# ahcorde/visualSLAM_Android

Hardware: AMD Instinct MI355X
Metric: frames/sec (TrackFrame+local BA) on 640×480 synthetic, 1/2/4/8 GPU (higher is better)
Workload: dtype f64

## Files before the change

visualslam_android_amd/csrc/patch_dev.h:

```cpp
#pragma once
#include "vslam_internal.h"

template <int PS> struct PRow { unsigned w[(PS + 3) / 4]; };
template <int PS> DEVFN PRow<PS> zero_row() {
  PRow<PS> r;
#pragma unroll
  for (int k = 0; k < (PS + 3) / 4; k++) r.w[k] = 0u;
  return r;
}
template <int PS> DEVFN PRow<PS> load_row(const uint8_t* p) {
  PRow<PS> r = zero_row<PS>();
  __builtin_memcpy(&r, p, PS);
  return r;
}
template <int PS> DEVFN PRow<PS> load_row_lds(const uint8_t* p) {
  PRow<PS> r = zero_row<PS>();
#pragma unroll
  for (int x = 0; x < PS; x++) r.w[x >> 2] |= (unsigned)p[x] << (8 * (x & 3));
  return r;
}
template <int PS> DEVFN int row_byte(const PRow<PS>& r, int x) { return (int)((r.w[x >> 2] >> (8 * (x & 3))) & 255u); }
DEVFN unsigned udot4(unsigned a, unsigned b, unsigned c) { return __builtin_amdgcn_udot4(a, b, c, false); }

template <int NPIX> DEVFN int zmssd_score(int tsum, int tsumsq, int sA, int sQ, int sX) {
  const int SA = tsum, SB = sA;
  return ((2 * SA * SB - SA * SA - SB * SB) / NPIX + sQ + tsumsq - 2 * sX);
}
template <int PS, int G> DEVFN void grp_zmssd_sums(const PRow<PS>& row, const PRow<PS>& trow, int& sA, int& sQ, int& sX) {
  unsigned a = 0, q = 0, x = 0;
#pragma unroll
  for (int k = 0; k < (PS + 3) / 4; k++) {
    a = udot4(row.w[k], 0x01010101u, a);
    q = udot4(row.w[k], row.w[k], q);
    x = udot4(row.w[k], trow.w[k], x);
  }
  sA = (int)grp_sum<G>(a); sQ = (int)grp_sum<G>(q); sX = (int)grp_sum<G>(x);
}
template <int PS>
DEVFN int wave_zmssd(const uint8_t* tmpl, const uint8_t* img, int ip, int wl, int hl, int cx, int cy, int tsum, int tsumsq, int max_ssd, int lane) {
  constexpr int NPIX = PS * PS, HALF = PS / 2;
  if (!(cx >= HALF && cy >= HALF && cx < wl - HALF && cy < hl - HALF)) return max_ssd + 1;
  int sA = 0, sQ = 0, sX = 0;
  for (int q = lane; q < NPIX; q += 64) {
    const int y = q / PS, x = q - y * PS;
    const int n = img[(size_t)(cy - HALF + y) * ip + (cx - HALF + x)], t = tmpl[q];
    sA += n; sQ += n * n; sX += n * t;
  }
  sA = wave_sum(sA); sQ = wave_sum(sQ); sX = wave_sum(sX);
  return zmssd_score<NPIX>(tsum, tsumsq, sA, sQ, sX);
}

DEVFN int search_level_and_warp(const Pose& pose, const double cam[3], const double d[4], const double right[3], const double down[3],
                                double warp_inv[4], int& search_level) {
  const double ooz = 1.0 / cam[2];
  double mr[3], md[3];
  pose_rot(pose, right, mr);
  pose_rot(pose, down, md);
  const double r0 = mr[0] - cam[0] * mr[2] * ooz, r1 = mr[1] - cam[1] * mr[2] * ooz;
  const double d0 = md[0] - cam[0] * md[2] * ooz, d1 = md[1] - cam[1] * md[2] * ooz;
  warp_inv[0] = (d[0] * r0 + d[1] * r1) * ooz; warp_inv[2] = (d[2] * r0 + d[3] * r1) * ooz;
  warp_inv[1] = (d[0] * d0 + d[1] * d1) * ooz; warp_inv[3] = (d[2] * d0 + d[3] * d1) * ooz;
  double det = warp_inv[0] * warp_inv[3] - warp_inv[1] * warp_inv[2];
  int lv = 0;
  while (det > 3 && lv < NLEV - 1) { lv++; det *= 0.25; }
  search_level = lv;
  return (det > 3 || det < 0.25) ? -1 : lv;
}

DEVFN void template_warp_matrix(const double warp_inv[4], int scale, double m2[4]) {
  double inv[4];
  inv2(warp_inv, inv);
  m2[0] = inv[0] * scale; m2[1] = inv[1] * scale; m2[2] = inv[2] * scale; m2[3] = inv[3] * scale;
}
DEVFN bool warp_moved(const double m2[4], const double last_warp[4]) {
  for (int i = 0; i < 2; i++) {
    const double dx = m2[i] - last_warp[i], dy = m2[2 + i] - last_warp[2 + i];
    if (dx * dx + dy * dy > 0.07 * 0.07) return true;
  }
  return false;
}
struct TemplateWarp {
  double across[2], down[2], cr[2], x0, y0;
  float x_bound, y_bound;
};
template <int PS> DEVFN TemplateWarp template_warp(const double m2[4], int irx, int iry, int iw, int ih) {
  constexpr int HALF = PS / 2;
  TemplateWarp w;
  w.across[0] = m2[0]; w.across[1] = m2[2]; w.down[0] = m2[1]; w.down[1] = m2[3];
  w.x0 = (double)irx - (m2[0] * HALF + m2[1] * HALF); w.y0 = (double)iry - (m2[2] * HALF + m2[3] * HALF);
  w.cr[0] = w.down[0] - PS * w.across[0]; w.cr[1] = w.down[1] - PS * w.across[1];
  w.x_bound = (float)(iw - 1); w.y_bound = (float)(ih - 1);
  return w;
}
DEVFN void warp_pixel_step(const TemplateWarp& w, double& x, double& y) { x += w.across[0]; y += w.across[1]; }
template <int PS> DEVFN void warp_row_step(const TemplateWarp& w, double& x, double& y) {
#pragma unroll
  for (int j = 0; j < PS; j++) warp_pixel_step(w, x, y);
  x += w.cr[0]; y += w.cr[1];
}
DEVFN int warp_sample(const TemplateWarp& w, const uint8_t* src, int sp, double x, double y, int& nOutside) {
  if (0 <= x && 0 <= y && x < w.x_bound && y < w.y_bound) {
    const int lx = (int)x, ly = (int)y;
    x -= lx; y -= ly;
    const uint8_t* q0 = src + (size_t)ly * sp + lx;
    return (uint8_t)((1 - y) * ((1 - x) * q0[0] + x * q0[1]) + y * ((1 - x) * q0[sp] + x * q0[sp + 1]));
  }
  nOutside++;
  return 0;
}

struct CoarseWindow {
  unsigned range;
  int top, bottom_plus_one, left, right;
  bool empty;
};
DEVFN CoarseWindow coarse_window(double irx, double iry, int range_l0, int scale, int rows) {
  CoarseWindow cw;
  cw.range = ((unsigned)range_l0 + scale - 1) / scale;
  cw.top = (int)(iry - cw.range);
// ... 39 lines not shown
```

visualslam_android_amd/csrc/track.hip:

```cpp
#include "vslam_internal.h"
#include "patch_dev.h"
#include "pvs_perm.h"

#define TRK_THREADS 256
#define SORT_CAP 4096
static_assert(SORT_CAP == PVS_SORT_CAP, "a level's list (at most max_points entries) fits the permutation's sort buffer");

template <class T>
DEVFN bool td_project(T& td, int& flags, const double* pos, const Pose& pose, const CamModel& cam, CamProj& pr) {
  flags &= ~TDF_IN_IMAGE;
  double c[3];
  pose_xform(pose, pos, c);
  td.cam[0] = c[0]; td.cam[1] = c[1]; td.cam[2] = c[2];
  if (c[2] < 0.001) return false;
  const double implane[2] = {c[0] / c[2], c[1] / c[2]};
  if (implane[0] * implane[0] + implane[1] * implane[1] > cam.largest_radius * cam.largest_radius) return false;
  pr = cam_project(cam, implane[0], implane[1]);
  td.image[0] = pr.im[0]; td.image[1] = pr.im[1];
  if (pr.invalid) return true;
  if (td.image[0] < 0 || td.image[1] < 0 || td.image[0] > cam.size[0] || td.image[1] > cam.size[1]) return true;
  flags |= TDF_IN_IMAGE;
  return true;
}

template <class T>
DEVFN void td_project_and_derivs(T& td, int& flags, const double* pos, const Pose& pose, const CamModel& cam) {
  CamProj pr;
  const bool projected = td_project(td, flags, pos, pose, cam, pr);
  if ((flags & TDF_FOUND) && projected) cam_derivs(cam, pr, td.derivs);
}

template <class T>
DEVFN void td_calc_jacobian(const T& td, double* jac) {
  const double ooz = 1.0 / td.cam[2];
  const double c[3] = {td.cam[0], td.cam[1], td.cam[2]};
  const double d0 = td.derivs[0], d1 = td.derivs[1], d2 = td.derivs[2], d3 = td.derivs[3];
#pragma unroll
  for (int m = 0; m < 6; m++) {
    double f0, f1;
    se3_generator_motion(m, c, ooz, f0, f1);
    jac[m] = d0 * f0 + d1 * f1;
    jac[6 + m] = d2 * f0 + d3 * f1;
  }
}

#ifdef VSLAM_PVS_OCC8
#define VSLAM_PVS_ATTR __attribute__((amdgpu_waves_per_eu(8, 8)))
#else
#define VSLAM_PVS_ATTR
#endif
#define PVS_OUT 13
struct PvsOut { double cam[3], image[2], derivs[4], warp_inv[4]; };
static_assert(sizeof(PvsOut) == PVS_OUT * 8 && sizeof(MapPointDev) == PVS_OUT * 8 && sizeof(MapPointDev) % 8 == 0, "one LDS buffer serves both directions");
static_assert(offsetof(TrackData, derivs) == 40 && offsetof(TrackData, warp_inv) == 96, "k_pvs's write-out indexes TrackData as doubles");
__global__ __launch_bounds__(64) void k_motion(MapDev m, int S, const double* sbi_rot ) {
  const int s = blockIdx.x * 64 + threadIdx.x;
  if (s >= S) return;
  if (!trk_in_step(m.held, s)) return;
  TrackerState* st = &m.st[s];
  const bool tracking = trk_runs_track_map(m.held, s, st);
  st->frame++;
  st->kf_pending = 0; st->kf_added = 0;
  if (!tracking) return;
  if (!st->recovered_now) {
    double v[6];
    for (int i = 0; i < 6; i++) v[i] = st->velocity[i];
    if (sbi_rot) { v[0] = 0.0; v[1] = 0.0; for (int i = 3; i < 6; i++) v[i] = sbi_rot[(size_t)s * 8 + i]; }
    const Pose pred = pose_mul(se3_exp(v), st->pose_final);
    st->start_pose = st->pose_final; st->pose_cur = pred;
  }
  for (int l = 0; l < NLEV; l++) { st->attempted[l] = 0; st->found[l] = 0; }
  st->n_search = 0; st->n_coarse = 0; st->n_iter = 0; st->n_l3 = 0; st->coarse_found = 0;
}

__global__ __launch_bounds__(TRK_THREADS) VSLAM_PVS_ATTR void k_pvs(MapDev m, TrackParams tp) {
  const int s = blockIdx.y;
  TrackerState* st = &m.st[s];
  const bool tracking = trk_runs_track_map(m.held, s, st);
  const int n_points = st->n_points, i0 = blockIdx.x * TRK_THREADS;
  if (!tracking || i0 >= n_points) return;
  __shared__ __align__(16) double pbuf[TRK_THREADS * PVS_OUT];
  __shared__ int wn[TRK_THREADS];
  const int nhere = min(TRK_THREADS, n_points - i0);
  {
    const double* src = (const double*)(m.pts + (size_t)s * tp.max_points + i0);
    for (int k = threadIdx.x; k < nhere * PVS_OUT; k += TRK_THREADS) pbuf[k] = src[k];
  }
  const Pose pred = st->pose_cur;
  __syncthreads();
  const int i = i0 + threadIdx.x;
  PvsOut td;
  int nwr = 0;
  if (i < n_points) {
    const MapPointDev p = *(const MapPointDev*)(pbuf + (size_t)threadIdx.x * PVS_OUT);
    const size_t gi = (size_t)s * tp.max_points + i;
    int level = -1;
    if (!p.bad) {
      int flags = m.pt_flags[gi];
      CamProj pr;
      const bool projected = td_project(td, flags, p.pos, pred, tp.cam, pr);
      nwr = projected ? 5 : 3;
      if (flags & TDF_IN_IMAGE) {
        nwr = PVS_OUT;
        cam_derivs(tp.cam, pr, td.derivs);
        int lv;
        level = search_level_and_warp(pred, td.cam, td.derivs, p.right, p.down, td.warp_inv, lv);
        if (level < 0) flags |= TDF_TMPL_BAD;
        else flags &= ~(TDF_SEARCHED | TDF_FOUND);
      }
      m.pt_flags[gi] = flags;
    }
    m.pt_level[gi] = level;
  }
  __syncthreads();
  wn[threadIdx.x] = nwr;
  {
    const double* t = (const double*)&td;
    for (int f = 0; f < PVS_OUT; f++) if (f < nwr) pbuf[threadIdx.x * PVS_OUT + f] = t[f];
  }
  __syncthreads();
  double* dst = (double*)(m.td + (size_t)s * tp.max_points + i0);
  for (int k = threadIdx.x; k < nhere * PVS_OUT; k += TRK_THREADS) {
    const int j = k / PVS_OUT, f = k - j * PVS_OUT;
    if (f < wn[j]) dst[(size_t)j * (sizeof(TrackData) / 8) + (f < 9 ? f : f + 3)] = pbuf[k];
  }
}

DEVFN int* pvs_chopped() { __shared__ int flag; return &flag; }
DEVFN uint64_t* pvs_sortbuf() { __shared__ uint64_t buf[SORT_CAP]; return buf; }
DEVFN void pvs_shuffle_list(uint64_t* buf, int* list, int n, uint64_t h, int L) {
  if (n < 2) return;
  pvs_block_fill<TRK_THREADS>(buf, n, h, L, nullptr);
  pvs_block_sort<TRK_THREADS>(buf, n);
  for (int j = threadIdx.x; j < n; j += TRK_THREADS) buf[j] = (uint64_t)(uint32_t)list[(uint32_t)buf[j]];
  __syncthreads();
  for (int j = threadIdx.x; j < n; j += TRK_THREADS) list[j] = (int)(uint32_t)buf[j];
  __syncthreads();
}

__device__ __attribute__((noinline)) void pvs_shuffle_levels(int* pvs, int P, const int* cnt, unsigned seed, int frame) {
  const uint64_t h = pvs_frame_hash(seed, frame);
  for (int l = 0; l < NLEV; l++) pvs_shuffle_list(pvs_sortbuf(), pvs + l * P, cnt[l], h, l);
}

template <bool SHUFFLE>
__global__ __launch_bounds__(TRK_THREADS) void k_plan(MapDev m, TrackParams tp, int stage) {
  const int s = blockIdx.x;
  TrackerState* st = &m.st[s];
  if (!trk_runs_track_map(m.held, s, st)) return;
  const int P = tp.max_points;
  TrackData* td = m.td + (size_t)s * P;
  const MapPointDev* pts = m.pts + (size_t)s * P;
  int* pvs = m.pvs_list + (size_t)s * NLEV * P;
  int2* slist = m.search_list + (size_t)s * P;
  int* ilist = m.iter_list + (size_t)s * P;
  const int lane = threadIdx.x & 63, wave = threadIdx.x >> 6;
  __shared__ int cnt[NLEV];
  __shared__ int wcnt[TRK_THREADS / 64][NLEV];
  __shared__ int plan[4];
  if (stage == 0) {
    if (threadIdx.x < NLEV) cnt[threadIdx.x] = 0;
    __syncthreads();
    const int n = st->n_points;
    constexpr int PLAN_CH = 16;
    for (int base = 0; base < n; base += PLAN_CH * TRK_THREADS) {
      const int first = base + threadIdx.x * PLAN_CH;
      int lv[PLAN_CH], c[NLEV] = {0, 0, 0, 0};
#pragma unroll
      for (int k = 0; k < PLAN_CH; k++) { const int i = first + k; lv[k] = m.pt_level[(size_t)s * P + (i < n ? i : n - 1)]; if (i >= n) lv[k] = -1; }
#pragma unroll
      for (int k = 0; k < PLAN_CH; k++)
#pragma unroll
        for (int l = 0; l < NLEV; l++) c[l] += lv[k] == l;
      int off[NLEV];
#pragma unroll
      for (int l = 0; l < NLEV; l++) {
        int inc = c[l];
        for (int d = 1; d < 64; d <<= 1) { const int t = __shfl_up(inc, d); if (lane >= d) inc += t; }
        if (lane == 63) wcnt[wave][l] = inc;
        off[l] = inc - c[l];
      }
      __syncthreads();
#pragma unroll
      for (int l = 0; l < NLEV; l++) { off[l] += cnt[l]; for (int w = 0; w < wave; w++) off[l] += wcnt[w][l]; }
#pragma unroll
      for (int k = 0; k < PLAN_CH; k++) {
#pragma unroll
        for (int l = 0; l < NLEV; l++) if (lv[k] == l) pvs[l * P + off[l]++] = first + k;
      }
      __syncthreads();
      if (threadIdx.x < NLEV) { int t = cnt[threadIdx.x]; for (int w = 0; w < TRK_THREADS / 64; w++) t += wcnt[w][threadIdx.x]; cnt[threadIdx.x] = t; }
      __syncthreads();
    }
    if constexpr (SHUFFLE) {
      const unsigned seed = st->pvs_seed;
      if (seed) pvs_shuffle_levels(pvs, P, cnt, seed, st->frame);
    }
    if (threadIdx.x == 0) {
      for (int l = 0; l < NLEV; l++) { st->pvs_count[l] = cnt[l]; st->pvs_head[l] = 0; }
      unsigned nCoarseMax = tp.coarse_max, nCoarseRange = tp.coarse_range;
      st->did_coarse = 0;
      bool bTry = true;
      if (tp.coarse_disabled || st->msd_vel < tp.coarse_min_vel || nCoarseMax == 0) bTry = false;
      if (st->just_recovered) { bTry = true; nCoarseMax *= 2; nCoarseRange *= 2; st->just_recovered = 0; }
      int c3 = 0, c2 = 0;
      const unsigned n3 = cnt[3], n2 = cnt[2];
      if (bTry && n3 + n2 > (unsigned)tp.coarse_min) {
        unsigned take3 = n3 <= nCoarseMax ? n3 : nCoarseMax;
        st->pvs_head[3] = take3;
        c3 = take3;
        if (take3 < nCoarseMax) {
          const unsigned more = nCoarseMax - take3;
          if (n2 <= more) { c3 = 0; c2 = n2; st->pvs_head[2] = n2; }
          else { c2 = more; st->pvs_head[2] = more; }
        }
      }
      plan[0] = c3; plan[1] = c2;
      st->coarse_range = nCoarseRange;
      st->n_coarse = c3 + c2; st->n_search = c3 + c2; st->n_iter = c3 + c2;
    }
    __syncthreads();
    const int c3 = plan[0], c2 = plan[1];
    for (int e = threadIdx.x; e < c3 + c2; e += TRK_THREADS) {
      const int idx = e < c3 ? pvs[3 * P + e] : pvs[2 * P + (e - c3)];
      slist[e] = make_int2(idx, tp.coarse_subpix_its);
      ilist[e] = idx;
    }
  } else {
    __shared__ Pose pose;
    if (threadIdx.x == 0) {
      pose = st->pose_cur;
      const int nit = st->n_iter;
      const int h3 = st->pvs_head[3], n3 = st->pvs_count[3] - h3;
      int nother = (st->pvs_count[2] - st->pvs_head[2]) + st->pvs_count[1] + st->pvs_count[0];
      int nFine = tp.max_patches - (nit + n3);
      if (nFine < 0) nFine = 0;
      if constexpr (SHUFFLE) *pvs_chopped() = nother > nFine && nFine > 0 && st->pvs_seed != 0;
      if (nother > nFine) nother = nFine;
      plan[0] = nit; plan[1] = n3; plan[2] = nother;
      st->fine_range = st->did_coarse ? 5 : 10;
      st->n_l3 = n3; st->n_search = n3 + nother; st->n_iter = nit + n3 + nother;
    }
    __syncthreads();
    const int nit = plan[0], n3 = plan[1], nother = plan[2];
    const int h3 = st->pvs_head[3], h2 = st->pvs_head[2];
    const int r2 = st->pvs_count[2] - h2, r1 = st->pvs_count[1];
    const int did_coarse = st->did_coarse;
    const uint64_t* rest_order = nullptr;
    if constexpr (SHUFFLE) {
      uint64_t* sortbuf = pvs_sortbuf();
      if (*pvs_chopped()) {
        const int nrest = r2 + r1 + st->pvs_count[0];
        pvs_block_fill<TRK_THREADS>(sortbuf, nrest, pvs_frame_hash(st->pvs_seed, st->frame), PVS_LIST_REST, nullptr);
        pvs_block_sort<TRK_THREADS>(sortbuf, nrest);
        rest_order = sortbuf;
      }
    }
    for (int e = threadIdx.x; e < n3 + nother; e += TRK_THREADS) {
      int idx, its;
      if (e < n3) { idx = pvs[3 * P + h3 + e]; its = tp.fine_subpix_its; }
      else {
        int k = e - n3;
        if constexpr (SHUFFLE) if (rest_order) k = (int)(uint32_t)rest_order[k];
        if (k < r2) idx = pvs[2 * P + h2 + k];
        else if (k < r2 + r1) idx = pvs[1 * P + (k - r2)];
        else idx = pvs[0 * P + (k - r2 - r1)];
        its = 0;
      }
      if (e < n3 || did_coarse) td_project_and_derivs(td[idx], m.pt_flags[(size_t)s * P + idx], pts[idx].pos, pose, tp.cam);
      slist[e] = make_int2(idx, its);
      ilist[nit + e] = idx;
    }
  }
}

struct SearchArgs {
  const uint8_t* img[NLEV]; size_t img_sstride[NLEV]; int img_pitch[NLEV];
  const uint32_t* corners[NLEV]; const int* rowlut[NLEV]; const int* ncorners;
  int w[NLEV], h[NLEV], cap[NLEV];
  size_t kf_stride[NLEV];
  int kf_pitch[NLEV];
  int nblk, S;
};


#define TRK_XCDS 8
DEVFN void xcd_stream_block(int nblk, int S, int& s, int& blk) {
  const int i = blockIdx.x, x = i % TRK_XCDS, j = i / TRK_XCDS;
  blk = j % nblk;
  s = (j / nblk) * TRK_XCDS + x;
  if (s >= S) s = -1;
}
static int xcd_grid(int nblk, int S) { return nblk * ((S + TRK_XCDS - 1) / TRK_XCDS) * TRK_XCDS; }

#ifndef SEARCH_N
#define SEARCH_N 128
#endif
#ifndef SEARCH_K
#define SEARCH_K 4
#endif
#ifdef VSLAM_BA_PROF
#define SEARCH_PROF_SLOTS 64
__device__ unsigned long long g_search_prof[2][SEARCH_PROF_SLOTS];
enum { SP_ENTRY, SP_TEMPLATE, SP_LUT, SP_FILTER, SP_ZMSSD, SP_WRITE, SP_PHASES };
#define SEARCH_PROF(...) __VA_ARGS__
#define SEARCH_PROF_BEGIN() const bool sp_on = (blockIdx.x / TRK_XCDS) % 7 == 0; unsigned long long sp_ph[SP_PHASES] = {0, 0, 0, 0, 0, 0}, sp_t0 = clock64(); \
  int sp_ftrips = 0, sp_ztrips = 0, sp_ncorners = 0; bool sp_refresh = false
#define SEARCH_STAMP(id) do { if (sp_on) { const unsigned long long t_ = clock64(); sp_ph[id] += t_ - sp_t0; sp_t0 = t_; } } while (0)
#define SEARCH_PROF_END() do { if (sp_on) search_prof_flush(g_search_prof[stage], sp_ph, sp_ftrips, sp_ztrips, sp_refresh, e < nsearch && lead, sp_ncorners, (int)nEval); } while (0)
DEVFN void search_prof_flush(unsigned long long* g, const unsigned long long* ph, int ftrips, int ztrips, bool refresh, bool patch, int ncorners, int nsurv) {
  if (threadIdx.x == 0) {
    for (int i = 0; i < SP_PHASES; i++) atomicAdd(&g[i], ph[i]);
    atomicAdd(&g[6], 1ull); atomicAdd(&g[7], refresh ? 1ull : 0ull); atomicAdd(&g[8], (unsigned long long)ftrips); atomicAdd(&g[9], (unsigned long long)ztrips);
    atomicAdd(&g[34 + (ftrips < 5 ? ftrips : 5)], 1ull); atomicAdd(&g[40 + (ztrips < 9 ? ztrips : 9)], 1ull);
  }
  if (patch) {
    atomicAdd(&g[10], (unsigned long long)((nsurv + SEARCH_K - 1) / SEARCH_K)); atomicAdd(&g[11], 1ull);
    atomicAdd(&g[12], (unsigned long long)nsurv); atomicAdd(&g[13], (unsigned long long)ncorners);
    const int cb = ncorners == 0 ? 0 : ncorners <= 64 ? 1 + (ncorners - 1) / 16 : ncorners <= 128 ? 5 + (ncorners - 65) / 32 : 7;
    const int sb = nsurv <= 4 ? nsurv : nsurv <= 16 ? 5 + (nsurv - 5) / 4 : 8;
    atomicAdd(&g[16 + cb], 1ull); atomicAdd(&g[24 + sb], 1ull);
  }
// ... 745 lines not shown
    int ta = 0, tf = 0, la = 0, lf = 0;
    for (int i = 0; i < NLEV; i++) { ta += st->attempted[i]; tf += st->found[i]; if (i >= 2) { la += st->attempted[i]; lf += st->found[i]; } }
    int quality;
    if (tf == 0 || ta == 0) quality = 0;
    else {
      const double dTotal = (double)tf / ta;
      const double dLarge = la > 10 ? (double)lf / la : dTotal;
      if (dTotal > 0.3) quality = 2; else if (dLarge < 0.13) quality = 0; else quality = 1;
    }
    if (quality == 1 && closest > tp.wiggle_scale * 10.0) quality = 0;
    if (quality == 0) st->lost_frames++; else st->lost_frames = 0;
    st->quality = quality;
  }
  if (!recovered) {
    double dDist = closest;
    dDist *= (1.0 / st->depth_mean);
    const bool need = dDist > tp.max_kf_dist_wiggle_mult * st->wiggle_depth_norm;
    if (st->quality == 2 && need && st->frame - st->last_kf_dropped > tp.min_frames_between_kf &&
        (st->n_kf < tp.max_keyframes || (tp.keyframe_retire && st->ba_countdown <= 0))) {
      st->kf_pending = 1;
      st->last_kf_dropped = st->frame;
    }
  }
  POSE_STAMP(9);
}

#ifdef VSLAM_BA_PROF
extern "C" int vslam_debug_search_prof(unsigned long long* out, int reset) {
  HIPCHK(hipDeviceSynchronize());
  HIPCHK(hipMemcpyFromSymbol(out, HIP_SYMBOL(g_search_prof), sizeof(unsigned long long) * 2 * SEARCH_PROF_SLOTS));
  if (reset) { unsigned long long z[2 * SEARCH_PROF_SLOTS] = {0}; HIPCHK(hipMemcpyToSymbol(HIP_SYMBOL(g_search_prof), z, sizeof(z))); }
  out[15] = SEARCH_N; out[SEARCH_PROF_SLOTS + 15] = SEARCH_K;
  return VSLAM_OK;
}
extern "C" int vslam_debug_pose_prof(unsigned long long* out16, int reset) {
  HIPCHK(hipDeviceSynchronize());
  HIPCHK(hipMemcpyFromSymbol(out16, HIP_SYMBOL(g_pose_prof), sizeof(unsigned long long) * 16));
  if (reset) { unsigned long long z[16] = {0}; HIPCHK(hipMemcpyToSymbol(HIP_SYMBOL(g_pose_prof), z, sizeof(z))); }
  return VSLAM_OK;
}
#endif

int trk_alloc(vslam_system* sys) {
  const vslam_params& p = sys->p;
  const size_t S = sys->S, P = p.max_points, K = p.max_keyframes;
  if (P > SORT_CAP) { vslam_set_error("max_points %d exceeds %d", (int)P, SORT_CAP); return VSLAM_E_INVALID; }
  MapDev& m = sys->map; DevOwner& own = sys->own; hipStream_t q = sys->stream;
  VCHK(own.alloc(&m.pts, S * P, q)); VCHK(own.alloc(&m.td, S * P, q)); VCHK(own.alloc(&m.tmpl, S * P * TMPL_PITCH, q));
  VCHK(own.alloc(&m.kf_meas, S * K * P, q)); VCHK(own.alloc(&m.cur_meas, S * P, q));
  VCHK(own.alloc(&m.kf_pose, S * K, q)); VCHK(own.alloc(&m.kf_fixed, S * K, q)); VCHK(own.alloc(&m.kf_depth, S * K * 2, q));
  for (int l = 0; l < NLEV; l++) VCHK(own.alloc(&m.kf_img[l], S * K * (size_t)sys->geom[l].pitch * sys->geom[l].h, q));
  VCHK(own.alloc(&m.st, S, q)); VCHK(own.alloc(&m.pvs_list, S * NLEV * P, q)); VCHK(own.alloc(&m.search_list, S * P, q)); VCHK(own.alloc(&m.iter_list, S * P, q)); VCHK(own.alloc(&m.pt_level, S * P, q)); VCHK(own.alloc(&m.pt_flags, S * P, q));
  VCHK(own.alloc(&m.pose_ws, S * POSE_WS_COMPS * P, q)); VCHK(own.alloc(&m.pose_wsi, S * 2 * P, q));
  trk_fill_params(p, sys->tp);
  return VSLAM_OK;
}

void cam_fill(CamModel& c, const double cam5[5], double width, double height, int quirks) {
  c.size[0] = width; c.size[1] = height;
  c.focal[0] = c.size[0] * cam5[0]; c.focal[1] = c.size[1] * cam5[1];
  c.center[0] = c.size[0] * cam5[2] - 0.5; c.center[1] = c.size[1] * cam5[3] - 0.5;
  c.w = cam5[4];
  double one_over_2tan = 0;
  if (c.w != 0.0) { c.two_tan = 2.0 * vlm::vtan(c.w / 2.0); one_over_2tan = 1.0 / c.two_tan; c.winv = 1.0 / c.w; c.distortion_enabled = 1.0; }
  else { c.winv = 0; c.two_tan = 0; c.distortion_enabled = 0; }
  double v2[2];
  if (quirks & VSLAM_Q_CAM_INT_RADIUS) {
    int m1 = (int)cam5[2], m2 = (int)(1.0 - cam5[2]);
    v2[0] = (m1 > m2 ? m1 : m2) / cam5[0];
    m1 = (int)cam5[3]; m2 = (int)(1.0 - cam5[3]);
    v2[1] = (m1 > m2 ? m1 : m2) / cam5[1];
  } else {
    v2[0] = (cam5[2] > 1.0 - cam5[2] ? cam5[2] : 1.0 - cam5[2]) / cam5[0];
    v2[1] = (cam5[3] > 1.0 - cam5[3] ? cam5[3] : 1.0 - cam5[3]) / cam5[1];
  }
  const double rr = sqrt(v2[0] * v2[0] + v2[1] * v2[1]);
  c.largest_radius = c.w == 0.0 ? rr : vlm::vtan(rr * c.w) * one_over_2tan;
  c.max_r = 1.5 * c.largest_radius;
}

void trk_fill_params(const vslam_params& p, TrackParams& t) {
  cam_fill(t.cam, p.cam, p.width, p.height, p.quirks);
  t.P = p.patch_size; t.max_ssd = 500 * p.patch_size * p.patch_size;
  t.max_patches = p.max_patches_per_frame; t.coarse_min = p.coarse_min; t.coarse_max = p.coarse_max; t.coarse_range = p.coarse_range;
  t.coarse_subpix_its = p.coarse_subpix_its; t.coarse_disabled = p.coarse_disabled; t.fine_subpix_its = p.fine_subpix_its;
  t.coarse_min_vel = p.coarse_min_vel; t.wls_prior = p.wls_prior;
  t.min_frames_between_kf = p.min_frames_between_kf; t.max_kf_dist_wiggle_mult = p.max_kf_dist_wiggle_mult; t.wiggle_scale = p.wiggle_scale;
  t.ba_max_iterations = p.ba_max_iterations; t.ba_convergence_limit = p.ba_convergence_limit;
  t.ba_min_sigma2 = p.ba_min_tukey_sigma * p.ba_min_tukey_sigma; t.ba_window = p.ba_window; t.ba_min_keyframes = p.ba_min_keyframes;
  t.quirks = p.quirks; t.max_points = p.max_points; t.max_keyframes = p.max_keyframes; t.ba_delay = p.ba_delay_frames;
  t.ba_batch = p.ba_batch_frames > 1 ? p.ba_batch_frames : 1;
  t.ba_sum_order = p.ba_sum_order ? 1 : 0;
  t.grow_map = p.grow_map;
  t.idle = p.idle_iterations != 0; t.fq_cap = 8192;
  t.keyframe_retire = p.keyframe_retire ? 1 : 0;
  {
    double a[2], b[2];
    cam_unproject(t.cam, t.cam.size[0] / 2, t.cam.size[1] / 2, a);
    cam_unproject(t.cam, t.cam.size[0] / 2 + 1, t.cam.size[1] / 2 + 1, b);
    const double d0 = a[0] - b[0], d1 = a[1] - b[1];
    t.one_pixel_dist = sqrt(d0 * d0 + d1 * d1) / sqrt(2.0);
  }
  const int kcap_max[NLEV] = {16384, 8192, 4096, 2048};
  for (int l = 0; l < NLEV; l++) t.kcap[l] = p.max_corners[l] < kcap_max[l] ? p.max_corners[l] : kcap_max[l];

}

static void trk_search_args(vslam_system* sys, SearchArgs& a) {
  for (int l = 0; l < NLEV; l++) {
    a.img[l] = sys->fr.img[l]; a.img_sstride[l] = sys->fr.img_sstride[l]; a.img_pitch[l] = sys->fr.img_pitch[l];
    a.corners[l] = sys->fr.corners[l]; a.rowlut[l] = sys->fr.rowlut[l];
    a.w[l] = sys->geom[l].w; a.h[l] = sys->geom[l].h; a.cap[l] = sys->geom[l].cap;
    a.kf_pitch[l] = sys->geom[l].pitch; a.kf_stride[l] = (size_t)sys->geom[l].pitch * sys->geom[l].h;
  }
  a.ncorners = sys->fr.ncorners;
}

typedef void (*PlanKernel)(MapDev, TrackParams, int);
static PlanKernel plan_kernel(const vslam_system* sys) { return sys->p.pvs_shuffle_seed ? k_plan<true> : k_plan<false>; }

int trk_search_stage(vslam_system* sys, int stage) {
  const int S = sys->S, P = sys->p.max_points;
  MapDev& m = sys->map;
  const TrackParams& tp = sys->tp;
  SearchArgs a;
  trk_search_args(sys, a);
  a.S = S; a.nblk = 1;
  if (stage == 0) {
    prof_mark(sys, PROF_PVS);
    overlay_note_track_map(sys);
    hipLaunchKernelGGL(k_motion, dim3((S + 63) / 64), dim3(64), 0, sys->stream, m, S, sys->p.use_sbi ? (const double*)sys->fr.sbi_rot : (const double*)nullptr);
// ... 99 lines not shown
```

visualslam_android_amd/csrc/vslam_internal.h:

```cpp
#pragma once
#include <hip/hip_runtime.h>
#include <stdint.h>
#include <string>
#include <vector>
#include "../../include/vslam_c.h"
#include "dev_math.h"

#define NLEV VSLAM_LEVELS

void vslam_set_error(const char* fmt, ...);

#define HIPCHK(expr)                                                                         \
  do {                                                                                       \
    hipError_t _e = (expr);                                                                  \
    if (_e != hipSuccess) {                                                                  \
      vslam_set_error("%s:%d: %s -> %s", __FILE__, __LINE__, #expr, hipGetErrorString(_e)); \
      return VSLAM_E_HIP;                                                                    \
    }                                                                                        \
  } while (0)

#define VCHK(expr) do { int _r = (expr); if (_r) return _r; } while (0)

static inline Pose pose_from12(const double* q) { Pose p; for (int i = 0; i < 9; i++) p.R[i] = q[i]; for (int i = 0; i < 3; i++) p.t[i] = q[9 + i]; return p; }
static inline void pose_to12(const Pose& p, double* q) { for (int i = 0; i < 9; i++) q[i] = p.R[i]; for (int i = 0; i < 3; i++) q[9 + i] = p.t[i]; }

struct LevelGeom {
  int w, h;
  int pitch;
  int nchunk;
  int cap;
  int thr;
};

struct FrameDev {
  const uint8_t* img[NLEV];
  size_t img_sstride[NLEV];
  int img_pitch[NLEV];
  unsigned long long* cmask[NLEV];
  int* rowcnt[NLEV];
  int* rowlut[NLEV];
  uint32_t* corners[NLEV];
  int* ncorners;
  int* overflow;
  int* scores[NLEV];
  uint32_t* maxcorners[NLEV];
  int* nmax;
  uint8_t* sbi_small;
  float* sbi_tmpl;
  float* sbi_jacs;
  double* sbi_rot;
  int* step_list;
  unsigned char* held;
};


#define POSE_WS_COMPS 12
#define TMPL_PITCH 128

struct MapPointDev {
  double pos[3], right[3], down[3];
  int src_kf, src_level, irx, iry;
  int bad, n_in, n_out, n_meas_kfs;
};

#define TDF_IN_IMAGE 1
#define TDF_FOUND 2
#define TDF_SEARCHED 4
#define TDF_SUBPIX 8
#define TDF_TMPL_BAD 16
#define TDF_HAVE_LAST 32

struct TrackData {
  double cam[3], image[2], derivs[4];
  double vfound[2], sqrt_inv_noise;
  double warp_inv[4], last_warp[4];
  int tsum, tsumsq;
};
// ... 49 lines not shown
DEVFN bool trk_runs_track_map(const unsigned char* held, int s, const TrackerState* st) {
  return trk_in_step(held, s) && st->map_good && (st->lost_frames < 3 || st->recovered_now);
}
DEVFN bool trk_kf_pending(const unsigned char* held, int s, const TrackerState* st) { return trk_in_step(held, s) && st->kf_pending; }

struct TrackParams {
  CamModel cam;
  int P;
  int max_ssd;
  int max_patches, coarse_min, coarse_max, coarse_range, coarse_subpix_its, coarse_disabled, fine_subpix_its;
  double coarse_min_vel, wls_prior;
  int min_frames_between_kf; double max_kf_dist_wiggle_mult, wiggle_scale;
  int ba_max_iterations; double ba_convergence_limit, ba_min_sigma2; int ba_window, ba_min_keyframes;
  int quirks;
  int max_points, max_keyframes;
  int ba_delay;
  int ba_batch;
  int ba_sum_order;
  int grow_map;
  int idle;
  int fq_cap;
  double one_pixel_dist;
  int kcap[NLEV];
  int keyframe_retire;
};

struct MapDev {
  MapPointDev* pts;
  TrackData* td;
  uint8_t* tmpl;
  MeasDev* kf_meas;
  MeasDev* cur_meas;
  Pose* kf_pose;
  int* kf_fixed;
  double* kf_depth;
  uint8_t* kf_img[NLEV];
  uint32_t* kf_corners[NLEV];
  int* kf_ncorners;
  unsigned long long* never_retry;
  int2* fq;
  uint8_t* trail_patch;
  int* trail_pos;
  double* boot_match;
  int* boot_inl;
  double* boot_ws;
  TrackerState* st;
  int* pvs_list;
  int2* search_list;
  int* pt_level;
  int* pt_flags;
  int* iter_list;
  double* pose_ws;
  int* pose_wsi;
  const unsigned char* held;
};

struct RelocInfo {
  int attempts, successes, best, frame;
  double best_zmssd, score;
  double ln_adj[6];
  Pose best_pose;
};
struct RelocDev {
  float* kf_tmpl;
  float* kf_jacs;
  float* cur_tmpl;
  double* scores;
  RelocInfo* info;
};

struct DevOwner {
  enum Kind : int { MEM, PINNED, STREAM, EVENT };
  struct Held { Kind kind; void* h; };
  std::vector<Held> held;
  template <class T> int alloc(T** out, size_t count, hipStream_t zero_on) {
    void* ptr = nullptr;
    HIPCHK(hipMalloc(&ptr, count * sizeof(T) + 64));
    held.push_back({MEM, ptr});
    HIPCHK(hipMemsetAsync(ptr, 0, count * sizeof(T) + 64, zero_on));
    *out = (T*)ptr;
    return VSLAM_OK;
  }
  int pinned(void** out, size_t bytes) {
    HIPCHK(hipHostMalloc(out, bytes, hipHostMallocDefault));
    held.push_back({PINNED, *out});
    return VSLAM_OK;
  }
  int stream(hipStream_t* out) {
    HIPCHK(hipStreamCreateWithFlags(out, hipStreamNonBlocking));
    held.push_back({STREAM, *out});
    return VSLAM_OK;
  }
  int event(hipEvent_t* out, bool timing) {
    HIPCHK(hipEventCreateWithFlags(out, timing ? hipEventDefault : hipEventDisableTiming));
    held.push_back({EVENT, *out});
    return VSLAM_OK;
  }
  void release() {
    for (const Held& x : held) if (x.kind == STREAM) (void)hipStreamSynchronize((hipStream_t)x.h);
    for (size_t i = held.size(); i-- > 0;) {
      const Held& x = held[i];
      if (x.kind == MEM) (void)hipFree(x.h);
      else if (x.kind == PINNED) (void)hipHostFree(x.h);
      else if (x.kind == EVENT) (void)hipEventDestroy((hipEvent_t)x.h);
      else (void)hipStreamDestroy((hipStream_t)x.h);
    }
// ... 125 lines not shown
  hipEvent_t ev_overlay_t[2] = {nullptr, nullptr};
  long overlay_calls = 0;
  hipEvent_t ev_snap_t[4] = {nullptr, nullptr, nullptr, nullptr};
  bool snap_timed[2] = {false, false};
  bool boot_key_pressed = false;
  std::vector<unsigned char> boot_key_stream;
  TrackParams tp;
  MapDev map;
  BaSystemWs* ba_ws = nullptr;
  RelocDev reloc = {nullptr, nullptr, nullptr, nullptr, nullptr};
  std::vector<hipEvent_t> prof_ev;
  int prof_cap = 0, prof_frame = 0;
  bool prof_on = false;
};

enum ProfStage : int {
  PROF_PYR_FAST0, PROF_FAST_LVL, PROF_COMPACT, PROF_PVS, PROF_PLAN_COARSE, PROF_SEARCH_COARSE, PROF_POSE_COARSE, PROF_PLAN_FINE,
  PROF_SEARCH_FINE, PROF_POSE_FINE, PROF_ADD_KEYFRAME, PROF_BA_ASSEMBLE, PROF_BA_COMPUTE, PROF_BA_WRITEBACK, PROF_FRAME_END
};
static_assert(PROF_FRAME_END == VSLAM_N_STAGES, "ProfStage names every stage of include/vslam_c.h");
#define PROF_MARKS (VSLAM_N_STAGES + 3)
#define PROF_FE_END (VSLAM_N_STAGES + 1)
#define PROF_BA_END (VSLAM_N_STAGES + 2)
static inline void prof_mark(vslam_system* sys, int k) {
  if (!(sys->prof_on && sys->prof_frame < sys->prof_cap)) return;
  hipStream_t st = sys->stream;
  if (k <= PROF_COMPACT || k == PROF_FE_END) st = sys->fe_stream;
  else if (sys->tp.ba_delay > 0 && (k == PROF_BA_COMPUTE || k == PROF_BA_END)) st = sys->ba_stream;
  (void)hipEventRecord(sys->prof_ev[(size_t)sys->prof_frame * PROF_MARKS + k], st);
}

int fe_make_keyframe_lite(vslam_system* sys, const uint8_t* gray, size_t row_stride, size_t stream_stride,
                          int on_device, const int* streams = nullptr, int n = -1);
int fe_stream_in_step(vslam_system* sys, int stream, const char* who);
int fe_fast_nonmax(vslam_system* sys);
int fe_keyframe_corners(vslam_system* sys, int s, int kf);
int fe_keyframe_rest_gated(vslam_system* sys);
int fe_thin_new_keyframe(vslam_system* sys, int level);
int grow_alloc(vslam_system* sys);
int grow_on_keyframe(vslam_system* sys);
enum IdleRefind : int { REFIND_NEWLY_MADE = 0, REFIND_FAILURE_QUEUE = 1 };
int grow_idle_refind(vslam_system* sys, int mode);
int mm_idle(vslam_system* sys);
int boot_alloc(vslam_system* sys);
int boot_frame(vslam_system* sys);
int grow_copy_corners(vslam_system* sys);
int grow_levels(vslam_system* sys, const int* order, int n);
int ba_launch_add_keyframe(vslam_system* sys);
enum IdleJob : int { IDLE_BA_RECENT = 0, IDLE_REFIND_NEW = 1, IDLE_BA_ALL = 2, IDLE_REFIND_FAILED = 3, IDLE_N_JOBS };
int mm_idle_job(vslam_system* sys, int job);
int fe_sbi(vslam_system* sys, const FrameDev& last, const int* list, int n);
int fe_sbi_carry(vslam_system* sys, const FrameDev& last);
int fe_sbi_restart(vslam_system* sys);
void cam_fill(CamModel& c, const double cam5[5], double width, double height, int quirks);
int fe_make_keyframe_rest(vslam_system* sys, double min_score);
int fe_thin_candidates(vslam_system* sys, int keyframe);
void trk_fill_params(const vslam_params& p, TrackParams& t);
int trk_alloc(vslam_system* sys);
int trk_track_map(vslam_system* sys);
int trk_search_stage(vslam_system* sys, int stage);
int trk_pose_stage(vslam_system* sys, int stage);
enum class BaJob : int {
  Keyframe = 0,
  Recent = 1,
  All = 2,
  IdleRecent = 3,
  IdleAll = 4,
  BootAll = 5,
  BootAllUntilConverged = 6,
};
enum class BaWriteback : int {
  Keyframe = 0,
  Recent = 1,
  All = 2,
  IfDue = 3,
  Drain = 4,
  Boot = 5,
};
constexpr bool ba_job_all(BaJob j) { return j == BaJob::All || j == BaJob::IdleAll || j >= BaJob::BootAll; }
constexpr bool ba_job_on_request(BaJob j) { return j == BaJob::Recent || j == BaJob::All; }
constexpr BaWriteback ba_job_writeback(BaJob j) {
  return j == BaJob::Keyframe ? BaWriteback::Keyframe : j >= BaJob::BootAll ? BaWriteback::Boot : ba_job_all(j) ? BaWriteback::All : BaWriteback::Recent;
}
DEVFN bool ba_job_gate(BaJob j, const TrackerState& st) {
  switch (j) {
    case BaJob::Keyframe: return st.kf_pending;
    case BaJob::IdleRecent: return !st.ba_converged_recent;
    case BaJob::IdleAll: return st.ba_converged_recent && !st.ba_converged_full;
    case BaJob::BootAll: return st.boot_run;
    case BaJob::BootAllUntilConverged: return st.boot_run && !st.ba_converged_full;
    default: return true;
  }
}
DEVFN int* ba_job_idle_counter(BaJob j, TrackerState* st) {
  return j == BaJob::IdleRecent ? &st->n_ba_recent_idle : j == BaJob::IdleAll ? &st->n_ba_all : nullptr;
}
int ba_alloc(vslam_system* sys);
void ba_free(vslam_system* sys);
int ba_add_keyframe_and_adjust(vslam_system* sys);
int ba_run(vslam_system* sys, BaJob job, bool host_driven_keyframe = false);
int ba_frame_start(vslam_system* sys);
int ba_sync_streams(vslam_system* sys);
int reloc_alloc(vslam_system* sys);
int reloc_keyframe_sbi_pending(vslam_system* sys);
int reloc_keyframe_sbi(vslam_system* sys, int s, int first, int n);
int reloc_attempt_recovery(vslam_system* sys);
int ba_reset_streams(vslam_system* sys, const unsigned char* d_flags);
// ... 12 lines not shown
```

Measured before the change: 538,200.

## Defer per-point track data writes to plan stage for selected points only

The potentially-visible-set kernel no longer writes projected camera coords, image position, derivatives and warp to TrackData for every map point. It only computes flags and search level. The plan stage recomputes and writes these fields just for the points it actually schedules for search, using a predicted pose stored per system. This is meant to remove the large strided LDS-staged write-out of TrackData for all points, at the cost of redundant projection math for selected points. It also moves some helpers to host-device headers.

```diff
diff --git a/visualslam_android_amd/csrc/patch_dev.h b/visualslam_android_amd/csrc/patch_dev.h
--- a/visualslam_android_amd/csrc/patch_dev.h
+++ b/visualslam_android_amd/csrc/patch_dev.h
@@ -50,8 +50,8 @@
   return zmssd_score<NPIX>(tsum, tsumsq, sA, sQ, sX);
 }
 
-DEVFN int search_level_and_warp(const Pose& pose, const double cam[3], const double d[4], const double right[3], const double down[3],
-                                double warp_inv[4], int& search_level) {
+HDFN int search_level_and_warp(const Pose& pose, const double cam[3], const double d[4], const double right[3], const double down[3],
+                               double warp_inv[4], int& search_level) {
   const double ooz = 1.0 / cam[2];
   double mr[3], md[3];
   pose_rot(pose, right, mr);
@@ -65,6 +65,39 @@
   while (det > 3 && lv < NLEV - 1) { lv++; det *= 0.25; }
   search_level = lv;
   return (det > 3 || det < 0.25) ? -1 : lv;
+}
+
+template <class T>
+HDFN bool td_project(T& td, int& flags, const double* pos, const Pose& pose, const CamModel& cam, CamProj& pr) {
+  flags &= ~TDF_IN_IMAGE;
+  double c[3];
+  pose_xform(pose, pos, c);
+  td.cam[0] = c[0]; td.cam[1] = c[1]; td.cam[2] = c[2];
+  if (c[2] < 0.001) return false;
+  const double implane[2] = {c[0] / c[2], c[1] / c[2]};
+  if (implane[0] * implane[0] + implane[1] * implane[1] > cam.largest_radius * cam.largest_radius) return false;
+  pr = cam_project(cam, implane[0], implane[1]);
+  td.image[0] = pr.im[0]; td.image[1] = pr.im[1];
+  if (pr.invalid) return true;
+  if (td.image[0] < 0 || td.image[1] < 0 || td.image[0] > cam.size[0] || td.image[1] > cam.size[1]) return true;
+  flags |= TDF_IN_IMAGE;
+  return true;
+}
+
+struct PvsOut { double cam[3], image[2], derivs[4], warp_inv[4]; };
+HDFN int pvs_point(const double pos[3], const double right[3], const double down[3], int bad, int& flags, const Pose& pred, const CamModel& cam, PvsOut& o) {
+  if (bad) return -1;
+  int level = -1;
+  CamProj pr;
+  td_project(o, flags, pos, pred, cam, pr);
+  if (flags & TDF_IN_IMAGE) {
+    cam_derivs(cam, pr, o.derivs);
+    int lv;
+    level = search_level_and_warp(pred, o.cam, o.derivs, right, down, o.warp_inv, lv);
+    if (level < 0) flags |= TDF_TMPL_BAD;
+    else flags &= ~(TDF_SEARCHED | TDF_FOUND);
+  }
+  return level;
 }
 
 DEVFN void template_warp_matrix(const double warp_inv[4], int scale, double m2[4]) {
diff --git a/visualslam_android_amd/csrc/track.hip b/visualslam_android_amd/csrc/track.hip
--- a/visualslam_android_amd/csrc/track.hip
+++ b/visualslam_android_amd/csrc/track.hip
@@ -5,23 +5,6 @@
 #define TRK_THREADS 256
 #define SORT_CAP 4096
 static_assert(SORT_CAP == PVS_SORT_CAP, "a level's list (at most max_points entries) fits the permutation's sort buffer");
-
-template <class T>
-DEVFN bool td_project(T& td, int& flags, const double* pos, const Pose& pose, const CamModel& cam, CamProj& pr) {
-  flags &= ~TDF_IN_IMAGE;
-  double c[3];
-  pose_xform(pose, pos, c);
-  td.cam[0] = c[0]; td.cam[1] = c[1]; td.cam[2] = c[2];
-  if (c[2] < 0.001) return false;
-  const double implane[2] = {c[0] / c[2], c[1] / c[2]};
-  if (implane[0] * implane[0] + implane[1] * implane[1] > cam.largest_radius * cam.largest_radius) return false;
-  pr = cam_project(cam, implane[0], implane[1]);
-  td.image[0] = pr.im[0]; td.image[1] = pr.im[1];
-  if (pr.invalid) return true;
-  if (td.image[0] < 0 || td.image[1] < 0 || td.image[0] > cam.size[0] || td.image[1] > cam.size[1]) return true;
-  flags |= TDF_IN_IMAGE;
-  return true;
-}
 
 template <class T>
 DEVFN void td_project_and_derivs(T& td, int& flags, const double* pos, const Pose& pose, const CamModel& cam) {
@@ -49,10 +32,9 @@
 #else
 #define VSLAM_PVS_ATTR
 #endif
-#define PVS_OUT 13
-struct PvsOut { double cam[3], image[2], derivs[4], warp_inv[4]; };
-static_assert(sizeof(PvsOut) == PVS_OUT * 8 && sizeof(MapPointDev) == PVS_OUT * 8 && sizeof(MapPointDev) % 8 == 0, "one LDS buffer serves both directions");
-static_assert(offsetof(TrackData, derivs) == 40 && offsetof(TrackData, warp_inv) == 96, "k_pvs's write-out indexes TrackData as doubles");
+#define PVS_IN 13
+static_assert(sizeof(MapPointDev) == PVS_IN * 8, "k_pvs stages map points as doubles");
+static_assert(sizeof(PvsOut) == 13 * 8 && offsetof(TrackData, image) == 24 && offsetof(TrackData, derivs) == 40 && offsetof(TrackData, warp_inv) == 96, "PvsOut names fields of a TrackData");
 __global__ __launch_bounds__(64) void k_motion(MapDev m, int S, const double* sbi_rot ) {
   const int s = blockIdx.x * 64 + threadIdx.x;
   if (s >= S) return;
@@ -69,6 +51,7 @@
     const Pose pred = pose_mul(se3_exp(v), st->pose_final);
     st->start_pose = st->pose_final; st->pose_cur = pred;
   }
+  m.pose_pred[s] = st->pose_cur;
   for (int l = 0; l < NLEV; l++) { st->attempted[l] = 0; st->found[l] = 0; }
   st->n_search = 0; st->n_coarse = 0; st->n_iter = 0; st->n_l3 = 0; st->coarse_found = 0;
 }
@@ -79,51 +62,23 @@
   const bool tracking = trk_runs_track_map(m.held, s, st);
   const int n_points = st->n_points, i0 = blockIdx.x * TRK_THREADS;
   if (!tracking || i0 >= n_points) return;
-  __shared__ __align__(16) double pbuf[TRK_THREADS * PVS_OUT];
-  __shared__ int wn[TRK_THREADS];
+  __shared__ __align__(16) double pbuf[TRK_THREADS * PVS_IN];
   const int nhere = min(TRK_THREADS, n_points - i0);
   {
     const double* src = (const double*)(m.pts + (size_t)s * tp.max_points + i0);
-    for (int k = threadIdx.x; k < nhere * PVS_OUT; k += TRK_THREADS) pbuf[k] = src[k];
-  }
-  const Pose pred = st->pose_cur;
+    for (int k = threadIdx.x; k < nhere * PVS_IN; k += TRK_THREADS) pbuf[k] = src[k];
+  }
+  const Pose pred = m.pose_pred[s];
   __syncthreads();
   const int i = i0 + threadIdx.x;
+  if (i >= n_points) return;
+  const MapPointDev p = *(const MapPointDev*)(pbuf + (size_t)threadIdx.x * PVS_IN);
+  const size_t gi = (size_t)s * tp.max_points + i;
+  int flags = p.bad ? 0 : m.pt_flags[gi];
   PvsOut td;
-  int nwr = 0;
-  if (i < n_points) {
-    const MapPointDev p = *(const MapPointDev*)(pbuf + (size_t)threadIdx.x * PVS_OUT);
-    const size_t gi = (size_t)s * tp.max_points + i;
-    int level = -1;
-    if (!p.bad) {
-      int flags = m.pt_flags[gi];
-      CamProj pr;
-      const bool projected = td_project(td, flags, p.pos, pred, tp.cam, pr);
-      nwr = projected ? 5 : 3;
-      if (flags & TDF_IN_IMAGE) {
-        nwr = PVS_OUT;
-        cam_derivs(tp.cam, pr, td.derivs);
-        int lv;
-        level = search_level_and_warp(pred, td.cam, td.derivs, p.right, p.down, td.warp_inv, lv);
-        if (level < 0) flags |= TDF_TMPL_BAD;
-        else flags &= ~(TDF_SEARCHED | TDF_FOUND);
-      }
-      m.pt_flags[gi] = flags;
-    }
-    m.pt_level[gi] = level;
-  }
-  __syncthreads();
-  wn[threadIdx.x] = nwr;
-  {
-    const double* t = (const double*)&td;
-    for (int f = 0; f < PVS_OUT; f++) if (f < nwr) pbuf[threadIdx.x * PVS_OUT + f] = t[f];
-  }
-  __syncthreads();
-  double* dst = (double*)(m.td + (size_t)s * tp.max_points + i0);
-  for (int k = threadIdx.x; k < nhere * PVS_OUT; k += TRK_THREADS) {
-    const int j = k / PVS_OUT, f = k - j * PVS_OUT;
-    if (f < wn[j]) dst[(size_t)j * (sizeof(TrackData) / 8) + (f < 9 ? f : f + 3)] = pbuf[k];
-  }
+  const int level = pvs_point(p.pos, p.right, p.down, p.bad, flags, pred, tp.cam, td);
+  if (!p.bad) m.pt_flags[gi] = flags;
+  m.pt_level[gi] = level;
 }
 
 DEVFN int* pvs_chopped() { __shared__ int flag; return &flag; }
@@ -141,6 +96,27 @@
 __device__ __attribute__((noinline)) void pvs_shuffle_levels(int* pvs, int P, const int* cnt, unsigned seed, int frame) {
   const uint64_t h = pvs_frame_hash(seed, frame);
   for (int l = 0; l < NLEV; l++) pvs_shuffle_list(pvs_sortbuf(), pvs + l * P, cnt[l], h, l);
+}
+
+DEVFN double uniform_double(double v) {
+  return __hiloint2double(__builtin_amdgcn_readfirstlane(__double2hiint(v)), __builtin_amdgcn_readfirstlane(__double2loint(v)));
+}
+DEVFN Pose uniform_pose(const Pose* p) {
+  Pose T;
+  for (int i = 0; i < 9; i++) T.R[i] = uniform_double(p->R[i]);
+  for (int i = 0; i < 3; i++) T.t[i] = uniform_double(p->t[i]);
+  return T;
+}
+DEVFN void plan_materialise(TrackData& t, const MapPointDev& p, int& flags, const Pose& pred, const Pose* cur, const CamModel& cam) {
+  double pos[3], right[3], down[3];
+  for (int i = 0; i < 3; i++) { pos[i] = p.pos[i]; right[i] = p.right[i]; down[i] = p.down[i]; }
+  PvsOut o;
+  int fl = 0;
+  pvs_point(pos, right, down, 0, fl, pred, cam, o);
+  if (cur) { fl = flags; td_project_and_derivs(o, fl, pos, *cur, cam); flags = fl; }
+  for (int i = 0; i < 3; i++) t.cam[i] = o.cam[i];
+  for (int i = 0; i < 2; i++) t.image[i] = o.image[i];
+  for (int i = 0; i < 4; i++) { t.derivs[i] = o.derivs[i]; t.warp_inv[i] = o.warp_inv[i]; }
 }
 
 template <bool SHUFFLE>
@@ -221,13 +197,16 @@
     }
     __syncthreads();
     const int c3 = plan[0], c2 = plan[1];
+    const Pose pred = uniform_pose(m.pose_pred + s);
     for (int e = threadIdx.x; e < c3 + c2; e += TRK_THREADS) {
       const int idx = e < c3 ? pvs[3 * P + e] : pvs[2 * P + (e - c3)];
+      plan_materialise(td[idx], pts[idx], m.pt_flags[(size_t)s * P + idx], pred, nullptr, tp.cam);
       slist[e] = make_int2(idx, tp.coarse_subpix_its);
       ilist[e] = idx;
     }
   } else {
     __shared__ Pose pose;
+    const Pose pred = uniform_pose(m.pose_pred + s);
     if (threadIdx.x == 0) {
       pose = st->pose_cur;
       const int nit = st->n_iter;
@@ -267,7 +246,7 @@
         else idx = pvs[0 * P + (k - r2 - r1)];
         its = 0;
       }
-      if (e < n3 || did_coarse) td_project_and_derivs(td[idx], m.pt_flags[(size_t)s * P + idx], pts[idx].pos, pose, tp.cam);
+      plan_materialise(td[idx], pts[idx], m.pt_flags[(size_t)s * P + idx], pred, e < n3 || did_coarse ? &pose : nullptr, tp.cam);
       slist[e] = make_int2(idx, its);
       ilist[nit + e] = idx;
     }
@@ -1119,31 +1098,9 @@
   for (int l = 0; l < NLEV; l++) VCHK(own.alloc(&m.kf_img[l], S * K * (size_t)sys->geom[l].pitch * sys->geom[l].h, q));
   VCHK(own.alloc(&m.st, S, q)); VCHK(own.alloc(&m.pvs_list, S * NLEV * P, q)); VCHK(own.alloc(&m.search_list, S * P, q)); VCHK(own.alloc(&m.iter_list, S * P, q)); VCHK(own.alloc(&m.pt_level, S * P, q)); VCHK(own.alloc(&m.pt_flags, S * P, q));
   VCHK(own.alloc(&m.pose_ws, S * POSE_WS_COMPS * P, q)); VCHK(own.alloc(&m.pose_wsi, S * 2 * P, q));
+  VCHK(own.alloc(&m.pose_pred, S, q));
   trk_fill_params(p, sys->tp);
   return VSLAM_OK;
-}
-
-void cam_fill(CamModel& c, const double cam5[5], double width, double height, int quirks) {
-  c.size[0] = width; c.size[1] = height;
-  c.focal[0] = c.size[0] * cam5[0]; c.focal[1] = c.size[1] * cam5[1];
-  c.center[0] = c.size[0] * cam5[2] - 0.5; c.center[1] = c.size[1] * cam5[3] - 0.5;
-  c.w = cam5[4];
-  double one_over_2tan = 0;
-  if (c.w != 0.0) { c.two_tan = 2.0 * vlm::vtan(c.w / 2.0); one_over_2tan = 1.0 / c.two_tan; c.winv = 1.0 / c.w; c.distortion_enabled = 1.0; }
-  else { c.winv = 0; c.two_tan = 0; c.distortion_enabled = 0; }
-  double v2[2];
-  if (quirks & VSLAM_Q_CAM_INT_RADIUS) {
-    int m1 = (int)cam5[2], m2 = (int)(1.0 - cam5[2]);
-    v2[0] = (m1 > m2 ? m1 : m2) / cam5[0];
-    m1 = (int)cam5[3]; m2 = (int)(1.0 - cam5[3]);
-    v2[1] = (m1 > m2 ? m1 : m2) / cam5[1];
-  } else {
-    v2[0] = (cam5[2] > 1.0 - cam5[2] ? cam5[2] : 1.0 - cam5[2]) / cam5[0];
-    v2[1] = (cam5[3] > 1.0 - cam5[3] ? cam5[3] : 1.0 - cam5[3]) / cam5[1];
-  }
-  const double rr = sqrt(v2[0] * v2[0] + v2[1] * v2[1]);
-  c.largest_radius = c.w == 0.0 ? rr : vlm::vtan(rr * c.w) * one_over_2tan;
-  c.max_r = 1.5 * c.largest_radius;
 }
 
 void trk_fill_params(const vslam_params& p, TrackParams& t) {
diff --git a/visualslam_android_amd/csrc/vslam_internal.h b/visualslam_android_amd/csrc/vslam_internal.h
--- a/visualslam_android_amd/csrc/vslam_internal.h
+++ b/visualslam_android_amd/csrc/vslam_internal.h
@@ -23,6 +23,29 @@
 
 static inline Pose pose_from12(const double* q) { Pose p; for (int i = 0; i < 9; i++) p.R[i] = q[i]; for (int i = 0; i < 3; i++) p.t[i] = q[9 + i]; return p; }
 static inline void pose_to12(const Pose& p, double* q) { for (int i = 0; i < 9; i++) q[i] = p.R[i]; for (int i = 0; i < 3; i++) q[9 + i] = p.t[i]; }
+
+inline void cam_fill(CamModel& c, const double cam5[5], double width, double height, int quirks) {
+  c.size[0] = width; c.size[1] = height;
+  c.focal[0] = c.size[0] * cam5[0]; c.focal[1] = c.size[1] * cam5[1];
+  c.center[0] = c.size[0] * cam5[2] - 0.5; c.center[1] = c.size[1] * cam5[3] - 0.5;
+  c.w = cam5[4];
+  double one_over_2tan = 0;
+  if (c.w != 0.0) { c.two_tan = 2.0 * vlm::vtan(c.w / 2.0); one_over_2tan = 1.0 / c.two_tan; c.winv = 1.0 / c.w; c.distortion_enabled = 1.0; }
+  else { c.winv = 0; c.two_tan = 0; c.distortion_enabled = 0; }
+  double v2[2];
+  if (quirks & VSLAM_Q_CAM_INT_RADIUS) {
+    int m1 = (int)cam5[2], m2 = (int)(1.0 - cam5[2]);
+    v2[0] = (m1 > m2 ? m1 : m2) / cam5[0];
+    m1 = (int)cam5[3]; m2 = (int)(1.0 - cam5[3]);
+    v2[1] = (m1 > m2 ? m1 : m2) / cam5[1];
+  } else {
+    v2[0] = (cam5[2] > 1.0 - cam5[2] ? cam5[2] : 1.0 - cam5[2]) / cam5[0];
+    v2[1] = (cam5[3] > 1.0 - cam5[3] ? cam5[3] : 1.0 - cam5[3]) / cam5[1];
+  }
+  const double rr = sqrt(v2[0] * v2[0] + v2[1] * v2[1]);
+  c.largest_radius = c.w == 0.0 ? rr : vlm::vtan(rr * c.w) * one_over_2tan;
+  c.max_r = 1.5 * c.largest_radius;
+}
 
 struct LevelGeom {
   int w, h;
@@ -178,6 +201,7 @@
   int* iter_list;
   double* pose_ws;
   int* pose_wsi;
+  Pose* pose_pred;
   const unsigned char* held;
 };
 
@@ -409,7 +433,6 @@
 int fe_sbi(vslam_system* sys, const FrameDev& last, const int* list, int n);
 int fe_sbi_carry(vslam_system* sys, const FrameDev& last);
 int fe_sbi_restart(vslam_system* sys);
-void cam_fill(CamModel& c, const double cam5[5], double width, double height, int quirks);
 int fe_make_keyframe_rest(vslam_system* sys, double min_score);
 int fe_thin_candidates(vslam_system* sys, int keyframe);
 void trk_fill_params(const vslam_params& p, TrackParams& t);
```

Result: no change. 537,100 (-0.2%).
